# oKatanaaa/Cython3DModelRenderer

Measured on NVIDIA B200. Metric: T-Rex 1024^2 frames/s, higher is better.
Workload: dtype f32

## Files before the change

cython3dmodelrenderer_b200/csrc/crender_b200.cu:

```cuda

#include <cuda.h>
#include <cuda_runtime.h>

#include <climits>
#include <cmath>
#include <cstdarg>
#include <cstdint>
#include <cstdio>
#include <cstdlib>
#include <cstring>
#include <new>
#include <atomic>
#include <mutex>
#include <thread>
#include <vector>

#include "crender_b200.h"

namespace {

constexpr int TW = 32;
constexpr int TH = 32;
constexpr int NT = 256;
#ifndef CRB_RT
// ... 205 lines not shown
    c[2] = (X.w * b1 + C1.z * b2) + C2.y * b3;
    if (F.flags & CRB_GURO) {
        const float dot = (__fadd_rn(0.0f, n[0] * F.light[0]) + n[1] * F.light[1]) + n[2] * F.light[2];
        const float nrm = sqrtf((n[0] * n[0] + n[1] * n[1]) + n[2] * n[2]);
        float s = dot / (nrm + 1e-6f);
        if (s < 0.0f) s = 0.0f;
        if (s > 1.0f) s = 1.0f;
        c[0] *= s; c[1] *= s; c[2] *= s;
    }
    return true;
}

__device__ __forceinline__ float background_color(const Frame &)
{
    return 0.0f;
}

__device__ __forceinline__ unsigned char to_u8(float c)
{
    return (unsigned char)(c >= -2147483648.0f && c < 2147483648.0f ? (int)c : INT_MIN);
}

__device__ __forceinline__ unsigned char *u8_pixel(const Frame &F, int view, int yl, int x)
{
    const int fr = F.row1 - F.row0 - 1 - yl;
    if (F.u8xN) {
        const int d = fr / F.u8xRows;
        return F.u8x[d] + (((long long)view * F.u8xRows + (fr - d * F.u8xRows)) * F.W + x) * 3;
    }
    return F.color_u8 + ((long long)view * F.slabPixels + (long long)fr * F.W + x) * 3;
}


__device__ __forceinline__ void stage_floats(const float *__restrict__ g, long long first, long long count, float *s)
{
    const float *src = g + first;
    if (count == (long long)NT * 9 && (reinterpret_cast<uintptr_t>(src) & 15u) == 0) {
        const float4 *s4 = reinterpret_cast<const float4 *>(src);
        const unsigned t = threadIdx.x;
        const float4 a = __ldg(s4 + t), b = __ldg(s4 + t + NT);
        float4 c = make_float4(0.f, 0.f, 0.f, 0.f);
        if (t < NT * 9 / 4 - 2 * NT) c = __ldg(s4 + t + 2 * NT);
        reinterpret_cast<float4 *>(s)[t] = a;
        reinterpret_cast<float4 *>(s)[t + NT] = b;
        if (t < NT * 9 / 4 - 2 * NT) reinterpret_cast<float4 *>(s)[t + 2 * NT] = c;
    } else if ((reinterpret_cast<uintptr_t>(src) & 15u) == 0) {
        const long long n4 = count >> 2;
        const float4 *s4 = reinterpret_cast<const float4 *>(src);
        for (long long i = threadIdx.x; i < n4; i += NT) reinterpret_cast<float4 *>(s)[i] = __ldg(s4 + i);
        for (long long i = (n4 << 2) + threadIdx.x; i < count; i += NT) s[i] = __ldg(src + i);
    } else {
        for (long long i = threadIdx.x; i < count; i += NT) s[i] = __ldg(src + i);
    }
}

__device__ __forceinline__ void tile_span(const Frame &F, unsigned bx, unsigned by, int &tx0, int &tx1, int &ty0, int &ty1)
{
    const int xl = bx & 0xFFFF, xr = bx >> 16, yt = by & 0xFFFF, yb = by >> 16;
    tx0 = xl / TW;
    tx1 = (xr - 1) / TW;
    ty0 = (yt - F.row0) / TH;
    ty1 = (yb - 1 - F.row0) / TH;
}

constexpr int BC_STAGES = 4;
constexpr unsigned BC_BYTES = NT * 9 * 4;

__device__ __forceinline__ void mbar_init(unsigned long long *bar, unsigned count)
{
    asm volatile("mbarrier.init.shared::cta.b64 [%0], %1;" ::"r"((unsigned)__cvta_generic_to_shared(bar)), "r"(count) : "memory");
}
__device__ __forceinline__ void mbar_wait(unsigned long long *bar, unsigned phase)
{
    const unsigned a = (unsigned)__cvta_generic_to_shared(bar);
    asm volatile(
        "{\n"
        ".reg .pred p;\n"
        "WAIT_%=:\n"
        "mbarrier.try_wait.parity.shared::cta.b64 p, [%0], %1;\n"
        "@p bra DONE_%=;\n"
        "bra WAIT_%=;\n"
        "DONE_%=:\n"
        "}\n" ::"r"(a), "r"(phase) : "memory");
}
__device__ __forceinline__ void bulk_load(void *smem_dst, const void *gmem_src, unsigned bytes, unsigned long long *bar)
{
    const unsigned d = (unsigned)__cvta_generic_to_shared(smem_dst), m = (unsigned)__cvta_generic_to_shared(bar);
    asm volatile("mbarrier.arrive.expect_tx.shared::cta.b64 _, [%0], %1;" ::"r"(m), "r"(bytes) : "memory");
    asm volatile("cp.async.bulk.shared::cluster.global.mbarrier::complete_tx::bytes [%0], [%1], %2, [%3];" ::"r"(d), "l"(gmem_src),
                 "r"(bytes), "r"(m) : "memory");
}

__device__ __forceinline__ unsigned block_compact(const bool flag, unsigned *wsum, unsigned &total)
{
    const unsigned lane = threadIdx.x & 31u, wid = threadIdx.x >> 5;
    const unsigned b = __ballot_sync(0xFFFFFFFFu, flag);
    if (lane == 0) wsum[wid] = __popc(b);
    __syncthreads();
    unsigned base = 0, tot = 0;
#pragma unroll
    for (int w = 0; w < NT / 32; ++w) {
        const unsigned c = wsum[w];
        if (w < (int)wid) base += c;
        tot += c;
    }
    total = tot;
    __syncthreads();
    return base + __popc(b & ((1u << lane) - 1u));
}

__device__ __forceinline__ void setup_chunk(const Frame &F, const int view, const long long chunk, const long long chunksPerView,
                                            float *sv, float *sn, float *sc, float *sM, unsigned char *slist, unsigned *wsum,
                                            const bool staged)
{
    const long long first = chunk * NT;
    const long long cnt = min((long long)NT, F.T - first);
    const bool banded = F.row0 > 0 || F.row1 < F.H;
    unsigned short *alive = F.alive + (long long)view * chunksPerView + chunk;
    if (!staged) {
        stage_floats(F.v, first * 9, cnt * 9, sv);
        if (!banded) stage_floats(F.n, first * 9, cnt * 9, sn);
    }
    if (F.views && threadIdx.x < 16) sM[threadIdx.x] = F.views[view * 16 + threadIdx.x];
    __syncthreads();
    int me = threadIdx.x < cnt ? (int)threadIdx.x : -1;
    unsigned kept = 0;
    if (!banded) {
        bool keep = false;
        if (me >= 0) {
            const float *q = sn + me * 9;
            float z0 = q[2], z1 = q[5], z2 = q[8];
            if (F.views) {
                z0 = (sM[6] * q[0] + sM[7] * q[1]) + sM[8] * q[2];
                z1 = (sM[6] * q[3] + sM[7] * q[4]) + sM[8] * q[5];
                z2 = (sM[6] * q[6] + sM[7] * q[7]) + sM[8] * q[8];
            }
            keep = !(((z0 + z1) + z2) >= 0.0f);
        }
        const unsigned pos = block_compact(keep, wsum, kept);
        if (kept == 0) {
            if (threadIdx.x == 0) *alive = 0;
            return;
        }
        if (keep) slist[pos] = (unsigned char)me;
        __syncthreads();
        me = threadIdx.x < kept ? (int)slist[threadIdx.x] : -1;
    }
    const bool valid = me >= 0;
    const int mi = valid ? me : 0;
    const long long tri = first + mi;
    const long long ridx = (long long)view * F.T + tri;
    float x[3], y[3], z[3];
#pragma unroll
    for (int k = 0; k < 3; ++k) {
        if (!valid) { x[k] = y[k] = z[k] = 1.0f; continue; }
        x[k] = sv[mi * 9 + k * 3 + 0];
        y[k] = sv[mi * 9 + k * 3 + 1];
        z[k] = sv[mi * 9 + k * 3 + 2];
        if (F.views) view_point(sM, x[k], y[k], z[k]);
        project_vertex(F.proj, x[k], y[k], z[k]);
    }

    float fxl = (float)F.W, fxr = 0.0f, fyt = (float)F.H, fyb = 0.0f;
#pragma unroll
    for (int k = 0; k < 3; ++k) {
        if (x[k] < fxl) fxl = x[k];
        if (x[k] > fxr) fxr = x[k];
        if (y[k] < fyt) fyt = y[k];
        if (y[k] > fyb) fyb = y[k];
    }
    int xl = clipi(ceil_to_int_ref(fxl), 0, F.W), xr = clipi(ceil_to_int_ref(fxr), 0, F.W);
    int yt = clipi(ceil_to_int_ref(fyt), 0, F.H), yb = clipi(ceil_to_int_ref(fyb), 0, F.H);
    yt = max(yt, F.row0);
    yb = min(yb, F.row1);
    bool drawn = valid && (xl < xr) && (yt < yb);
    if (banded) {
        if (!__syncthreads_or(drawn ? 1 : 0)) {
            if (threadIdx.x == 0) *alive = 0;
            return;
        }
        if (!staged) {
            stage_floats(F.n, first * 9, cnt * 9, sn);
            __syncthreads();
        }
    }
    if (banded && valid) {
        const float *q = sn + mi * 9;
        float z0 = q[2], z1 = q[5], z2 = q[8];
        if (F.views) {
            z0 = (sM[6] * q[0] + sM[7] * q[1]) + sM[8] * q[2];
            z1 = (sM[6] * q[3] + sM[7] * q[4]) + sM[8] * q[5];
            z2 = (sM[6] * q[6] + sM[7] * q[7]) + sM[8] * q[8];
        }
        drawn = drawn && !(((z0 + z1) + z2) >= 0.0f);
    }
    const unsigned bx = drawn ? ((unsigned)xl | ((unsigned)xr << 16)) : 0u;
    const unsigned by = drawn ? ((unsigned)yt | ((unsigned)yb << 16)) : 0u;

    float l03 = 0.f, l13 = 0.f, l23 = 0.f;
    unsigned fl = 0;
    if (drawn) {
    l03 = (x[1] - x[2]) * (y[0] - y[2]) - (y[1] - y[2]) * (x[0] - x[2]);
    l13 = (x[2] - x[0]) * (y[1] - y[0]) - (y[2] - y[0]) * (x[1] - x[0]);
    l23 = (x[0] - x[1]) * (y[2] - y[1]) - (y[0] - y[1]) * (x[2] - x[1]);
    const float a03 = fabsf(l03), a13 = fabsf(l13), a23 = fabsf(l23);
    if (a03 >= L3_MIN && a03 <= L3_MAX) fl |= (FL_REJ << 0) | (l03 < 0.f ? (FL_NEG << 0) : 0u);
    if (a13 >= L3_MIN && a13 <= L3_MAX) fl |= (FL_REJ << 1) | (l13 < 0.f ? (FL_NEG << 1) : 0u);
    if (a23 >= L3_MIN && a23 <= L3_MAX) fl |= (FL_REJ << 2) | (l23 < 0.f ? (FL_NEG << 2) : 0u);
    float cmax = 0.0f;
#pragma unroll
    for (int k = 0; k < 3; ++k) cmax = fmaxf(cmax, fmaxf(fabsf(x[k]), fabsf(y[k])));
    const bool finite_xy = (x[0] - x[0] == 0.f) && (x[1] - x[1] == 0.f) && (x[2] - x[2] == 0.f) && (y[0] - y[0] == 0.f) &&
                           (y[1] - y[1] == 0.f) && (y[2] - y[2] == 0.f);
    if ((fl & (7u * FL_REJ)) == 7u * FL_REJ && finite_xy && cmax <= SPAN_COORD_MAX) fl |= FL_SPAN;
    if (fminf(fminf(a03, a13), a23) >= FDIV_LO && fmaxf(fmaxf(a03, a13), a23) <= FDIV_HI) fl |= FL_FDIV;
    }

    unsigned n_entries, dpos;
    bool entry;
    if (banded) {
        dpos = block_compact(drawn, wsum, n_entries);
        entry = drawn;
    } else {
        dpos = threadIdx.x; entry = valid;
        n_entries = __syncthreads_or(drawn ? 1 : 0) ? kept : 0u;
    }
    if (entry && n_entries) F.recE[(long long)view * F.T + first + dpos] = make_float4(__uint_as_float(bx), __uint_as_float(by), __uint_as_float((unsigned)mi), __uint_as_float(fl));
    if (threadIdx.x == 0) *alive = (unsigned short)n_entries;
    if (n_entries == 0) return;
    if (!staged) {
        stage_floats(F.c, first * 9, cnt * 9, sc);
        __syncthreads();
    }
    if (drawn) {
    float4 *R = F.shrec + ridx * SREC;
    const float *q = sc + mi * 9;
    R[S_A] = make_float4(x[0], y[0], x[1], y[1]);
    R[S_B] = make_float4(x[2], y[2], z[0], z[1]);
    R[S_C] = make_float4(z[2], l03, l13, l23);
    float nx[3], ny[3], nz[3];
#pragma unroll
    for (int k = 0; k < 3; ++k) {
        nx[k] = sn[mi * 9 + k * 3 + 0];
        ny[k] = sn[mi * 9 + k * 3 + 1];
        nz[k] = sn[mi * 9 + k * 3 + 2];
        if (F.views) view_normal(sM, nx[k], ny[k], nz[k]);
    }
    R[S_N0] = make_float4(nx[0], ny[0], nz[0], nx[1]);
    R[S_N1] = make_float4(ny[1], nz[1], nx[2], ny[2]);
    R[S_X] = make_float4(nz[2], q[0], q[1], q[2]);
    R[S_C1] = make_float4(q[3], q[4], q[5], q[6]);
    R[S_C2] = make_float4(q[7], q[8], __uint_as_float(fl), 0.0f);
    }
    if (F.flags & CRB_PATH_ATOMIC) return;

    int tx0 = 0, tx1 = -1, ty0 = 0, ty1 = -1;
    if (drawn) tile_span(F, bx, by, tx0, tx1, ty0, ty1);
    unsigned *cnt_view = F.count + (long long)view * F.nTiles;
    const int nt = drawn ? (tx1 - tx0 + 1) * (ty1 - ty0 + 1) : 0;
    if (nt <= WIDE_TILES)
        for (int ty = ty0; ty <= ty1; ++ty)
            for (int tx = tx0; tx <= tx1; ++tx) atomicAdd(cnt_view + ty * F.tilesX + tx, 1u);
    for (unsigned wide = __ballot_sync(0xFFFFFFFFu, nt > WIDE_TILES); wide; wide &= wide - 1u) {
        const int src = __ffs(wide) - 1;
        const int sx0 = __shfl_sync(0xFFFFFFFFu, tx0, src), sx1 = __shfl_sync(0xFFFFFFFFu, tx1, src);
        const int sy0 = __shfl_sync(0xFFFFFFFFu, ty0, src), n = __shfl_sync(0xFFFFFFFFu, nt, src);
        const int wx = sx1 - sx0 + 1;
        for (int i = (int)(threadIdx.x & 31u); i < n; i += 32) atomicAdd(cnt_view + (sy0 + i / wx) * F.tilesX + sx0 + i % wx, 1u);
    }
}

#ifndef CRB_SETUP_MIN_CTAS
#define CRB_SETUP_MIN_CTAS 3
#endif
constexpr int SETUP_STAGES = 2;
constexpr size_t SETUP_STAGE_FLOATS = 3 * (size_t)NT * 9;
constexpr size_t SETUP_DYN_SMEM = SETUP_STAGES * SETUP_STAGE_FLOATS * sizeof(float);
__global__ void __launch_bounds__(NT, CRB_SETUP_MIN_CTAS) k_setup(const Frame F)
{
    extern __shared__ __align__(128) float stg[];
    __shared__ __align__(8) unsigned long long bar[SETUP_STAGES];
    __shared__ float sM[16];
    __shared__ unsigned char slist[NT];
    __shared__ unsigned wsum[NT / 32];
    if (blockIdx.x == 0 && threadIdx.x == 0) {
        F.total[0] = 0ull; F.total[2] = 0ull; F.total[3] = 0ull; F.total[4] = 0ull; F.total[5] = 0ull;
    }
    const long long chunksPerView = (F.T + NT - 1) / NT;
    const long long nItems = F.chunks ? (long long)F.chunks[0] : chunksPerView * F.nViews;
    const bool banded = F.row0 > 0 || F.row1 < F.H;
    const bool bulk_ok = !((reinterpret_cast<uintptr_t>(F.v) | reinterpret_cast<uintptr_t>(F.n) | reinterpret_cast<uintptr_t>(F.c)) & 15u) &&
                         (!banded || F.chunks);
    auto item = [&](long long w, int &view) -> long long {
        if (F.chunks) { view = 0; return (long long)F.chunks[1 + w]; }
        view = (int)(w / chunksPerView);
        return w % chunksPerView;
    };
    auto issue = [&](long long w, int s) {
        int view;
        const long long chunk = item(w, view);
        if (!bulk_ok || (chunk + 1) * NT > F.T) return;
        float *d = stg + (size_t)s * SETUP_STAGE_FLOATS;
        bulk_load(d, F.v + chunk * NT * 9, BC_BYTES, &bar[s]);
        bulk_load(d + NT * 9, F.n + chunk * NT * 9, BC_BYTES, &bar[s]);
        bulk_load(d + 2 * NT * 9, F.c + chunk * NT * 9, BC_BYTES, &bar[s]);
    };
    if (threadIdx.x == 0) {
        for (int s = 0; s < SETUP_STAGES; ++s) mbar_init(&bar[s], 3u);
        asm volatile("fence.mbarrier_init.release.cluster;" ::: "memory");
        for (int s = 0; s < SETUP_STAGES; ++s)
            if ((long long)blockIdx.x + (long long)s * gridDim.x < nItems) issue((long long)blockIdx.x + (long long)s * gridDim.x, s);
    }
    __syncthreads();
    unsigned uses = 0;
    int i = 0;
    for (long long w = blockIdx.x; w < nItems; w += gridDim.x, ++i) {
        const int s = i % SETUP_STAGES;
        int view;
        const long long chunk = item(w, view);
        const bool staged = bulk_ok && (chunk + 1) * NT <= F.T;
        if (staged) {
            mbar_wait(&bar[s], (uses >> s) & 1u);
            uses ^= 1u << s;
        }
        float *d = stg + (size_t)s * SETUP_STAGE_FLOATS;
        setup_chunk(F, view, chunk, chunksPerView, d, d + NT * 9, d + 2 * NT * 9, sM, slist, wsum, staged);
        __syncthreads();
        const long long w2 = w + (long long)SETUP_STAGES * gridDim.x;
        if (threadIdx.x == 0 && w2 < nItems) issue(w2, s);
    }
}

__global__ void __launch_bounds__(NT) k_band_chunks(const Frame F)
{
    __shared__ __align__(128) float sv[BC_STAGES][NT * 9];
    __shared__ __align__(8) unsigned long long bar[BC_STAGES];
    const long long nFull = F.T / NT;
    if (blockIdx.x == 0 && threadIdx.x == 0 && nFull * NT < F.T) F.chunks[1 + atomicAdd(F.chunks, 1u)] = (unsigned)nFull;
    const long long nMine = nFull > blockIdx.x ? (nFull - blockIdx.x + gridDim.x - 1) / gridDim.x : 0;
    if (threadIdx.x == 0) {
        for (int s = 0; s < BC_STAGES; ++s) mbar_init(&bar[s], 1u);
        asm volatile("fence.mbarrier_init.release.cluster;" ::: "memory");
        for (int j = 0; j < BC_STAGES && j < nMine; ++j)
            bulk_load(sv[j], F.v + (blockIdx.x + (long long)j * gridDim.x) * (NT * 9), BC_BYTES, &bar[j]);
    }
    __syncthreads();
    for (long long j = 0; j < nMine; ++j) {
        const int s = (int)(j % BC_STAGES);
        mbar_wait(&bar[s], (unsigned)((j / BC_STAGES) & 1));
        float ylo = 3.0e38f, yhi = -3.0e38f;
        bool odd = false;
#pragma unroll
        for (int k = 0; k < 3; ++k) {
            const float vx = sv[s][threadIdx.x * 9 + k * 3 + 0];
            const float vy = sv[s][threadIdx.x * 9 + k * 3 + 1];
            const float vz = sv[s][threadIdx.x * 9 + k * 3 + 2];
            const float X = ((vx * F.proj.p[0] + vy * F.proj.p[4]) + vz * F.proj.p[8]) + F.proj.p[12];
            const float Y = ((X * F.proj.p[1] + vy * F.proj.p[5]) + vz * F.proj.p[9]) + F.proj.p[13];
            float r;
            asm("rcp.approx.ftz.f32 %0, %1;" : "=f"(r) : "f"(vz));
            const float ysc = (Y * r + 1.0f) * F.proj.ys;
            if (!(fabsf(ysc) < 1.0e9f)) odd = true;
// ... 52 lines not shown
    unsigned nheavyTiles;
    const unsigned htile = block_exclusive_scan(heavy ? 1u : 0u, warp_sums, nheavyTiles);
    __shared__ unsigned heavy_base;
    if (threadIdx.x == 0) {
        const unsigned valid = (unsigned)min((long long)NT, nAll - (long long)blockIdx.x * NT);
        block_base = tot ? atomicAdd(F.total, (unsigned long long)tot) : 0ull;
        busy_base = (unsigned)atomicAdd(F.total + 2, (unsigned long long)(nbusy - nheavyTiles));
        heavy_base = (unsigned)atomicAdd(F.total + 4, (unsigned long long)nheavy);
        empty_base = (unsigned)atomicAdd(F.total + 3, (unsigned long long)(valid - nbusy));
    }
    __syncthreads();
    if (i < nAll) {
        const unsigned long long o = block_base + excl;
        const unsigned o32 = (unsigned)(o > 0xFFFFFFFFull ? 0xFFFFFFFFull : o);
        F.offset[i] = o32;
        F.cursor[i] = 0u;
        F.count[i] = 0u;
        const unsigned vw = (unsigned)(i / F.nTiles), tl = (unsigned)(i % F.nTiles);
        const unsigned packed = (vw << 22) | ((tl / (unsigned)F.tilesX) << 11) | (tl % (unsigned)F.tilesX);
        constexpr unsigned FULL = (unsigned)TH << 8;
        if (cut)
            for (unsigned b = 0; b < (unsigned)SPLIT_BANDS; ++b)
                F.busyH[heavy_base + hrank + b] = make_uint4(packed, c, o32, (b * (TH / SPLIT_BANDS)) | (((b + 1) * (TH / SPLIT_BANDS)) << 8));
        else if (heavy) F.busyH[heavy_base + hrank] = make_uint4(packed, c, o32, FULL);
        else if (c) F.busy[busy_base + (brank - htile)] = make_uint4(packed, c, o32, FULL);
        else F.empty[empty_base + (threadIdx.x - brank)] = packed;
    }
}

constexpr int FT = 64;
__device__ __forceinline__ void fill_chunk(const Frame &F, const int view, const long long chunk, const long long chunksPerView, const bool skip,
                                           const unsigned tix )
{
    const long long slot = chunk * NT + tix;
    const float4 E = slot < F.T ? F.recE[(long long)view * F.T + slot] : make_float4(0.f, 0.f, 0.f, 0.f);
    const unsigned nd = F.alive[(long long)view * chunksPerView + chunk];
    if (skip || (tix & ~31u) >= nd) return;
    const unsigned bx = tix < nd ? __float_as_uint(E.x) : 0u, by = tix < nd ? __float_as_uint(E.y) : 0u;
    const bool drawn = (bx >> 16) != 0;
    const long long tri = chunk * NT + (drawn ? (long long)(__float_as_uint(E.z) & 255u) : 0ll);
    const long long ridx = (long long)view * F.T + tri;
    float4 a = make_float4(0.f, 0.f, 0.f, 0.f), b = a, s2 = a, s3 = a;
    int tx0 = 0, tx1 = -1, ty0 = 0, ty1 = -1;
    if (drawn) {
        const float4 *R = F.shrec + ridx * SREC;
        const float4 c = R[S_C];
        a = R[S_A]; b = R[S_B];
        const unsigned fl = __float_as_uint(E.w);
        s2 = make_float4(c.x, (fl & (FL_NEG << 0)) ? -c.y : c.y, (fl & (FL_NEG << 1)) ? -c.z : c.z, (fl & (FL_NEG << 2)) ? -c.w : c.w);
        s3 = make_float4(__uint_as_float(bx), __uint_as_float(by), __uint_as_float((unsigned)tri), __uint_as_float(fl));
        tile_span(F, bx, by, tx0, tx1, ty0, ty1);
    }
    const long long vb = (long long)view * F.nTiles;
    const int nt = drawn ? (tx1 - tx0 + 1) * (ty1 - ty0 + 1) : 0;
    {
        const unsigned lane = tix & 31u;
        const int small = nt <= WIDE_TILES ? nt : 0;
        const int turns = __reduce_max_sync(0xFFFFFFFFu, small);
        int cx = tx0, cy = ty0;
        for (int k = 0; k < turns; ++k) {
            const bool act = k < small;
            const long long t = vb + cy * F.tilesX + cx;
            const unsigned tag = act ? (unsigned)t : 0xFFFFFFE0u + lane;
            const unsigned grp = __match_any_sync(0xFFFFFFFFu, tag);
            const int leader = __ffs(grp) - 1;
            unsigned base = 0;
            if (act && (int)lane == leader) base = F.offset[t] + atomicAdd(F.cursor + t, (unsigned)__popc(grp));
            base = __shfl_sync(0xFFFFFFFFu, base, leader);
            if (act) {
                float4 *o = F.ls + (size_t)(base + __popc(grp & ((1u << lane) - 1u))) * 4;
                o[0] = a; o[1] = b; o[2] = s2; o[3] = s3;
                if (++cx > tx1) { cx = tx0; ++cy; }
            }
        }
    }
    unsigned widem = __ballot_sync(0xFFFFFFFFu, nt > WIDE_TILES);
    if (F.wideCap && widem) {
        const unsigned lane = tix & 31u;
        unsigned long long first = 0ull;
        if ((int)lane == __ffs(widem) - 1) first = atomicAdd(F.total + 5, (unsigned long long)__popc(widem));
        first = __shfl_sync(0xFFFFFFFFu, first, __ffs(widem) - 1);
        const unsigned long long at = first + __popc(widem & ((1u << lane) - 1u));
        const bool listed = nt > WIDE_TILES && at < (unsigned long long)F.wideCap;
        if (listed) F.wide[at] = make_uint4((unsigned)view, (unsigned)tri, bx, by);
        widem = __ballot_sync(0xFFFFFFFFu, nt > WIDE_TILES && !listed);
    }
    for (unsigned wide = widem; wide; wide &= wide - 1u) {
        const int src = __ffs(wide) - 1;
        auto bc = [src](float4 v) {
            return make_float4(__shfl_sync(0xFFFFFFFFu, v.x, src), __shfl_sync(0xFFFFFFFFu, v.y, src), __shfl_sync(0xFFFFFFFFu, v.z, src),
                               __shfl_sync(0xFFFFFFFFu, v.w, src));
        };
        const float4 wa = bc(a), wb = bc(b), w2 = bc(s2), w3 = bc(s3);
        const int sx0 = __shfl_sync(0xFFFFFFFFu, tx0, src), sx1 = __shfl_sync(0xFFFFFFFFu, tx1, src);
        const int sy0 = __shfl_sync(0xFFFFFFFFu, ty0, src), n = __shfl_sync(0xFFFFFFFFu, nt, src);
        const int wx = sx1 - sx0 + 1;
        for (int i = (int)(tix & 31u); i < n; i += 32) {
            const long long t = vb + (sy0 + i / wx) * F.tilesX + sx0 + i % wx;
            const unsigned at = F.offset[t] + atomicAdd(F.cursor + t, 1u);
            float4 *o = F.ls + (size_t)at * 4;
            o[0] = wa; o[1] = wb; o[2] = w2; o[3] = w3;
        }
    }
}

#ifndef CRB_FILL_MIN_CTAS
#define CRB_FILL_MIN_CTAS 16
#endif
__global__ void __launch_bounds__(FT, CRB_FILL_MIN_CTAS) k_fill(const Frame F)
{
    const long long chunksPerView = (F.T + NT - 1) / NT;
    const unsigned tix = (blockIdx.x & (NT / FT - 1)) * FT + threadIdx.x;
    if (!F.chunks) {
        fill_chunk(F, blockIdx.y, blockIdx.x / (NT / FT), chunksPerView, *F.total > (unsigned long long)F.pairCap, tix);
        return;
    }
    if (*F.total > (unsigned long long)F.pairCap) return;
    const unsigned n = F.chunks[0];
    for (unsigned i = blockIdx.x / (NT / FT); i < n; i += gridDim.x / (NT / FT)) fill_chunk(F, 0, F.chunks[1 + i], chunksPerView, false, tix);
}

constexpr int FWT = 256;
__global__ void __launch_bounds__(FWT) k_fill_wide(const Frame F)
{
    if (*F.total > (unsigned long long)F.pairCap) return;
    const unsigned long long listed = F.total[5];
    const unsigned n = (unsigned)(listed < (unsigned long long)F.wideCap ? listed : (unsigned long long)F.wideCap);
    for (unsigned e = blockIdx.x; e < n; e += gridDim.x) {
        const uint4 w = F.wide[e];
        const long long ridx = (long long)w.x * F.T + w.y;
        const float4 *R = F.shrec + ridx * SREC;
        const float4 a = R[S_A], b = R[S_B], c = R[S_C];
        const unsigned fl = __float_as_uint(R[S_C2].z);
        const float4 s2 = make_float4(c.x, (fl & (FL_NEG << 0)) ? -c.y : c.y, (fl & (FL_NEG << 1)) ? -c.z : c.z, (fl & (FL_NEG << 2)) ? -c.w : c.w);
        const float4 s3 = make_float4(__uint_as_float(w.z), __uint_as_float(w.w), __uint_as_float(w.y), __uint_as_float(fl));
        int tx0, tx1, ty0, ty1;
        tile_span(F, w.z, w.w, tx0, tx1, ty0, ty1);
        const int wx = tx1 - tx0 + 1, nt = wx * (ty1 - ty0 + 1);
        const long long vb = (long long)w.x * F.nTiles;
        for (int i0 = (int)threadIdx.x; i0 < nt; i0 += 4 * FWT) {
// ... 561 lines not shown

#ifdef CRB_LARGE_OUT_STAGE
constexpr bool LARGE_OUT_STAGE = true;
#else
constexpr bool LARGE_OUT_STAGE = false;
#endif
typedef RasterShape<CRB_RT, CRB_CH, CRB_FQ, CRB_CLEAR_ROWS, CRB_RASTER_MIN_CTAS, LARGE_OUT_STAGE> RasterLarge;
#ifndef CRB_SMALL_RT
#define CRB_SMALL_RT 128
#endif
#ifndef CRB_SMALL_CH
#define CRB_SMALL_CH 24
#endif
#ifndef CRB_SMALL_FQ
#define CRB_SMALL_FQ 256
#endif
#ifndef CRB_SMALL_CLEAR_ROWS
#define CRB_SMALL_CLEAR_ROWS 8
#endif
#ifndef CRB_SMALL_MIN_CTAS
#define CRB_SMALL_MIN_CTAS 12
#endif
typedef RasterShape<CRB_SMALL_RT, CRB_SMALL_CH, CRB_SMALL_FQ, CRB_SMALL_CLEAR_ROWS, CRB_SMALL_MIN_CTAS, false> RasterSmall;
typedef RasterShape<256, 128, 256, 16, 6, false> RasterWide;
#ifndef CRB_SHAPE_LARGE_FROM
#define CRB_SHAPE_LARGE_FROM 64
#endif

__global__ void __launch_bounds__(NT) k_raster_atomic(const Frame F, unsigned long long *keybuf)
{
    const long long slot = ((long long)blockIdx.x * NT + threadIdx.x) >> 5;
    const int lane = threadIdx.x & 31;
    if (slot >= F.T || (unsigned)(slot % NT) >= F.alive[slot / NT]) return;
    const float4 r2 = F.recE[slot];
    const unsigned bx = __float_as_uint(r2.x), by = __float_as_uint(r2.y);
    if ((bx >> 16) == 0) return;
    const long long tri = slot / NT * NT + (__float_as_uint(r2.z) & 255u);
    const Tri9 t = load_tri9(F, tri);
    const int xl = bx & 0xFFFF, xr = bx >> 16, yt = by & 0xFFFF, yb = by >> 16;
    const int bw = xr - xl;
    const long long area = (long long)bw * (yb - yt);
    for (long long i = lane; i < area; i += 32) {
        const int x = xl + (int)(i % bw), y = yt + (int)(i / bw);
        float b1, b2, b3;
        barycentric(t, (float)x, (float)y, b1, b2, b3);
        if (b1 < 0.0f || b2 < 0.0f || b3 < 0.0f) continue;
        const float z = (t.z0 * b1 + t.z1 * b2) + t.z2 * b3;
        if (z != z) continue;
        atomicMin(keybuf + (long long)(y - F.row0) * F.W + x, pack_key(z, (unsigned)tri));
    }
}

__global__ void __launch_bounds__(NT) k_shade_atomic(const Frame F, unsigned long long *keybuf)
{
    const long long pix = (long long)blockIdx.x * NT + threadIdx.x;
    if (pix >= F.slabPixels) return;
    const unsigned long long key = keybuf[pix];
    const bool clear = (F.flags & CRB_CLEAR_FIRST) != 0;
    float z = Z_INIT, c[3] = {0.f, 0.f, 0.f}, nn[3] = {0.f, 0.f, 0.f};
    bool write = clear;
    if (key != KEY_EMPTY) {
        keybuf[pix] = KEY_EMPTY;
        const unsigned tri = ~(unsigned)(key & 0xFFFFFFFFull);
        const int y = F.row0 + (int)(pix / F.W), x = (int)(pix % F.W);
        float fz, fc[3], fn[3];
        if (shade_fragment(F, F.shrec + (size_t)tri * SREC, (float)x, (float)y, fz, fc, fn)) {
            const float zold = clear ? Z_INIT : F.z[pix];
            if (!(fz > zold)) {
                z = fz; c[0] = fc[0]; c[1] = fc[1]; c[2] = fc[2]; nn[0] = fn[0]; nn[1] = fn[1]; nn[2] = fn[2];
                write = true;
// ... 249 lines not shown
    unsigned long long *hstats;
    unsigned long long *hstats_dev;
    bool prof_on;
    int prof_n;
    cudaEvent_t *prof_ev;
    int wide_kernel;
    unsigned char *u8x[CRB_MAX_EXCHANGE];
    int u8x_n, u8x_rows;
};

namespace {

struct WsLayout {
    size_t shrec, recE, alive, chunks, count, offset, cursor, busy, busyH, empty, ls, wide, total, set_bytes, sv, sc, sn, bytes;
};

long long default_pair_cap(const crb_filler *f, long long T, int views)
{
    const long long tiles = (long long)((f->w + TW - 1) / TW) * ((f->row1 - f->row0 + TH - 1) / TH);
    long long cap = 4 * T * views + tiles * views + 65536;
    return cap;
}

long long wide_capacity(long long T, int views) { return (T > 0 ? T : 1) * views / 8 + 1024; }

WsLayout ws_layout(const crb_filler *f, long long T, int views, long long pairCap)
{
    WsLayout L;
    const long long tiles = (long long)((f->w + TW - 1) / TW) * ((f->row1 - f->row0 + TH - 1) / TH);
    size_t o = 0;
    auto take = [&](size_t bytes) { size_t at = o; o = align_up(o + bytes, 256); return at; };
    const size_t recs = (size_t)(T > 0 ? T : 1) * views;
    L.shrec = take(recs * SREC * sizeof(float4));
    L.recE = take(recs * sizeof(float4));
    L.alive = take((size_t)((T > 0 ? T : 1) + NT - 1) / NT * views * sizeof(unsigned short));
    L.chunks = take(4 * ((size_t)((T > 0 ? T : 1) + NT - 1) / NT + 2));
    L.count = take((size_t)tiles * views * 4);
    L.offset = take((size_t)tiles * views * 4);
    L.cursor = take((size_t)tiles * views * 4);
    L.busy = take((size_t)tiles * views * 16);
    L.busyH = take((size_t)tiles * views * 16 * SPLIT_BANDS);
    L.empty = take((size_t)tiles * views * 4);
    L.ls = take((size_t)pairCap * 64);
    L.wide = take((size_t)wide_capacity(T, views) * 16);
    L.total = take(64);
    L.set_bytes = o;
    o = 2 * L.set_bytes;
    L.sv = take((size_t)(T > 0 ? T : 1) * 36);
    L.sc = take((size_t)(T > 0 ? T : 1) * 36);
    L.sn = take((size_t)(T > 0 ? T : 1) * 36);
    L.bytes = o;
    return L;
}

int check_filler(const crb_filler *f)
{
    if (!f) return fail(CRB_ERR_INVALID, "filler is NULL");
    return CRB_OK;
}

int check_triangles(const crb_filler *f, int64_t T, const float *v, const float *c, const float *n)
{
    if (T < 0) return fail(CRB_ERR_INVALID, "T < 0");
    if (T > 0 && (!v || !c || !n)) return fail(CRB_ERR_INVALID, "NULL triangle array");
    if (!f->ws) return fail(CRB_ERR_STATE, "workspace not bound");
    if (T > f->maxT) return fail(CRB_ERR_STATE, "T=%lld exceeds the workspace's max_triangles=%lld", (long long)T, f->maxT);
    if (T > 0xFFFFFFF0ll) return fail(CRB_ERR_INVALID, "T exceeds 32-bit triangle indices");
// ... 103 lines not shown
    return CRB_OK;
}

#ifndef CRB_PREPASS_EIGHTHS
#define CRB_PREPASS_EIGHTHS 5
#endif
int run_prep(crb_filler *f, Frame &F, cudaStream_t st, int slot = 0)
{
    int rc;
    bool wide_kernel = false;
    if (f->hstats && f->wide_kernel) {
        const unsigned long long hs = *reinterpret_cast<volatile unsigned long long *>(f->hstats + HSTAT_WORDS * (slot & 7));
        const unsigned long long hw = *reinterpret_cast<volatile unsigned long long *>(f->hstats + HSTAT_WORDS * (slot & 7) + 1) >> 32;
        wide_kernel = hs == 0ull || hw >= 24ull * (unsigned long long)F.nViews;
    }
    F.wideCap = wide_kernel && !(F.flags & CRB_PATH_ATOMIC) ? (unsigned)(f->wideCap > 0xFFFFFFF0ll ? 0xFFFFFFF0ll : f->wideCap) : 0u;
    unsigned gT = (unsigned)((F.T + NT - 1) / NT);
    const bool banded = F.row0 > 0 || F.row1 < F.H;
    F.chunks = nullptr;
    if (banded && f->band_prepass && 8ll * (F.row1 - F.row0) <= (long long)CRB_PREPASS_EIGHTHS * F.H && F.nViews == 1 && !F.views && F.T >= 8 * NT && !(F.flags & CRB_PATH_ATOMIC) &&
        !(reinterpret_cast<uintptr_t>(F.v) & 15u)) {
        const size_t so = (size_t)(reinterpret_cast<const char *>(F.alive) - reinterpret_cast<const char *>(f->alive));
        F.chunks = reinterpret_cast<unsigned *>(reinterpret_cast<char *>(f->chunks) + so);
        CU(cudaMemsetAsync(F.chunks, 0, 4, st));
        constexpr int bcPerSm = 4;
        const unsigned gP = (unsigned)min((long long)gT, (long long)f->sm_count * bcPerSm);
        k_band_chunks<<<gP, NT, 0, st>>>(F);
        if ((rc = launch_check(f, "k_band_chunks"))) return rc;
        gT = (unsigned)min((long long)gT, (long long)f->sm_count * 6);
    }
    if (F.T > 0) {
        if ((rc = setup_smem_attr(f->device))) return rc;
        const long long items = F.chunks ? (long long)gT : (long long)gT * F.nViews;
        k_setup<<<(unsigned)min(items, (long long)f->sm_count * CRB_SETUP_MIN_CTAS), NT, SETUP_DYN_SMEM, st>>>(F);
        if ((rc = launch_check(f, "k_setup"))) return rc;
    } else {
        CU(cudaMemsetAsync(F.total, 0, 8, st));
        CU(cudaMemsetAsync(F.total + 2, 0, 24, st));
    }
    F.splitHeavy = (F.nViews == 1 && f->split_heavy && F.nTiles <= 4 * f->sm_count * 6) ? 1u : 0u;
    const long long nAllTiles = (long long)F.nViews * F.nTiles;
    k_alloc<<<(unsigned)((nAllTiles + NT - 1) / NT), NT, 0, st>>>(F);
    if ((rc = launch_check(f, "k_alloc"))) return rc;
    if (F.T > 0) {
        k_fill<<<dim3(gT * (NT / FT), F.nViews), FT, 0, st>>>(F);
        if ((rc = launch_check(f, "k_fill"))) return rc;
        if (F.wideCap) {
            k_fill_wide<<<(unsigned)f->sm_count * 6, FWT, 0, st>>>(F);
            if ((rc = launch_check(f, "k_fill_wide"))) return rc;
        }
    }
    return CRB_OK;
}

int run_raster(crb_filler *f, Frame &F, cudaStream_t st, int slot)
{
    int rc;
    slot &= 7;
    if (F.hstats) F.hstats += HSTAT_WORDS * slot;
    const long long nAllTiles = (long long)F.nViews * F.nTiles;
    const bool prof = f->prof_on && f->prof_n < PROF_MAX;
    int shape = f->raster_shape;
    if (shape == 0) {
        const long long wave = (long long)f->sm_count * RasterWide::MIN_CTAS;
        double busy = (double)nAllTiles, per_tile = (double)F.T * 2.0 / (double)F.nTiles;
        if (f->hstats) {
            const unsigned long long hs = *reinterpret_cast<volatile unsigned long long *>(f->hstats + HSTAT_WORDS * slot);
// ... 39 lines not shown
    if (prof) CU(cudaEventRecord(f->prof_ev[2 * f->prof_n], st));
    if (shape == 2) k_raster<RasterSmall><<<(unsigned)gR, RasterSmall::RT, 0, st>>>(F, M);
    else if (shape == 3) k_raster<RasterWide><<<(unsigned)gR, RasterWide::RT, 0, st>>>(F, M);
    else k_raster<RasterLarge><<<(unsigned)gR, RasterLarge::RT, 0, st>>>(F, M);
    if ((rc = launch_check(f, "k_raster"))) return rc;
    if (prof) {
        CU(cudaEventRecord(f->prof_ev[2 * f->prof_n + 1], st));
        f->prof_n++;
    }
    return CRB_OK;
}

int run_tiled(crb_filler *f, Frame &F, cudaStream_t st, int slot = 0)
{
    int rc = run_prep(f, F, st, slot);
    return rc ? rc : run_raster(f, F, st, slot);
}

int run_atomic(crb_filler *f, Frame &F, cudaStream_t st)
{
    int rc;
    if (F.nViews != 1 || F.views) return fail(CRB_ERR_INVALID, "CRB_PATH_ATOMIC supports single-view renders only");
    if (!F.z || !F.color || !F.normals) return fail(CRB_ERR_STATE, "CRB_PATH_ATOMIC needs all three buffers");
    if (f->keybuf_pixels < F.slabPixels) {
        if (f->keybuf) cudaFree(f->keybuf);
        f->keybuf = nullptr;
        CU(cudaMalloc(&f->keybuf, (size_t)F.slabPixels * 8));
        f->keybuf_pixels = F.slabPixels;
        k_fill_u64<<<1184, NT, 0, st>>>(f->keybuf, F.slabPixels, KEY_EMPTY);
        if ((rc = launch_check(f, "k_fill_u64"))) return rc;
    }
    if (F.T > 0) {
        if ((rc = setup_smem_attr(f->device))) return rc;
        k_setup<<<(unsigned)min((F.T + NT - 1) / NT, (long long)f->sm_count * CRB_SETUP_MIN_CTAS), NT, SETUP_DYN_SMEM, st>>>(F);
        if ((rc = launch_check(f, "k_setup"))) return rc;
        k_raster_atomic<<<(unsigned)((F.T * 32 + NT - 1) / NT), NT, 0, st>>>(F, f->keybuf);
        if ((rc = launch_check(f, "k_raster_atomic"))) return rc;
    }
    k_shade_atomic<<<(unsigned)((F.slabPixels + NT - 1) / NT), NT, 0, st>>>(F, f->keybuf);
    return launch_check(f, "k_shade_atomic");
}

int join_pending(crb_filler *f, cudaStream_t st)
{
    if (f->pending_join) {
        CU(cudaStreamWaitEvent(st, f->ev_raster[f->pending_join - 1], 0));
        f->pending_join = 0;
    }
    return CRB_OK;
}

int bind_ws_pointers(crb_filler *f, void *ws, size_t bytes, long long T, int views, long long pairCap, cudaStream_t st)
{
    if (views < 1) views = 1;
    if (views > 1024) return fail(CRB_ERR_INVALID, "max_views > 1024 (views per launch; crb_render_views chunks longer batches itself)");
    if (T < 0) return fail(CRB_ERR_INVALID, "max_triangles < 0");
    if (pairCap <= 0) pairCap = default_pair_cap(f, T, views);
    if (pairCap > 0xFFFFFFF0ll) return fail(CRB_ERR_INVALID, "pair capacity exceeds 32-bit list offsets");
    const WsLayout L = ws_layout(f, T, views, pairCap);
    if (!ws || bytes < L.bytes) return fail(CRB_ERR_INVALID, "workspace too small: %zu < %zu", bytes, L.bytes);
    if (reinterpret_cast<uintptr_t>(ws) & 255u) return fail(CRB_ERR_INVALID, "workspace must be 256-byte aligned");
    char *b = (char *)ws;
    f->ws = ws; f->ws_bytes = bytes;
    f->maxT = T; f->maxViews = views; f->pairCap = pairCap;
    f->shrec = (float4 *)(b + L.shrec); f->recE = (float4 *)(b + L.recE);
    f->alive = (unsigned short *)(b + L.alive);
    f->chunks = (unsigned *)(b + L.chunks);
// ... 906 lines not shown
```

Baseline: 129,300.

## Restructure setup kernel into warp-independent culling with compact fat fill records

The setup kernel moves to 128-thread blocks in which each warp culls and sets up 64 triangles on its own. Block-wide compaction and __syncthreads are replaced by warp ballots plus a shared atomic counter, and the last warp to finish refills the stage. Color is no longer bulk-staged and is read directly from global memory. Setup now writes a 4-float4 compacted record holding geometry and the global triangle index, so the fill and atomic kernels read it directly instead of gathering from shrec. This removes block barriers and gather indirection, at the cost of a 4x larger recE buffer, more global writes, and reordered entry slots (the atomic order is nondeterministic).

```diff
diff --git a/cython3dmodelrenderer_b200/csrc/crender_b200.cu b/cython3dmodelrenderer_b200/csrc/crender_b200.cu
--- a/cython3dmodelrenderer_b200/csrc/crender_b200.cu
+++ b/cython3dmodelrenderer_b200/csrc/crender_b200.cu
@@ -261,28 +261,6 @@
 }
 
 
-__device__ __forceinline__ void stage_floats(const float *__restrict__ g, long long first, long long count, float *s)
-{
-    const float *src = g + first;
-    if (count == (long long)NT * 9 && (reinterpret_cast<uintptr_t>(src) & 15u) == 0) {
-        const float4 *s4 = reinterpret_cast<const float4 *>(src);
-        const unsigned t = threadIdx.x;
-        const float4 a = __ldg(s4 + t), b = __ldg(s4 + t + NT);
-        float4 c = make_float4(0.f, 0.f, 0.f, 0.f);
-        if (t < NT * 9 / 4 - 2 * NT) c = __ldg(s4 + t + 2 * NT);
-        reinterpret_cast<float4 *>(s)[t] = a;
-        reinterpret_cast<float4 *>(s)[t + NT] = b;
-        if (t < NT * 9 / 4 - 2 * NT) reinterpret_cast<float4 *>(s)[t + 2 * NT] = c;
-    } else if ((reinterpret_cast<uintptr_t>(src) & 15u) == 0) {
-        const long long n4 = count >> 2;
-        const float4 *s4 = reinterpret_cast<const float4 *>(src);
-        for (long long i = threadIdx.x; i < n4; i += NT) reinterpret_cast<float4 *>(s)[i] = __ldg(s4 + i);
-        for (long long i = (n4 << 2) + threadIdx.x; i < count; i += NT) s[i] = __ldg(src + i);
-    } else {
-        for (long long i = threadIdx.x; i < count; i += NT) s[i] = __ldg(src + i);
-    }
-}
-
 __device__ __forceinline__ void tile_span(const Frame &F, unsigned bx, unsigned by, int &tx0, int &tx1, int &ty0, int &ty1)
 {
     const int xl = bx & 0xFFFF, xr = bx >> 16, yt = by & 0xFFFF, yb = by >> 16;
@@ -312,69 +290,30 @@
         "DONE_%=:\n"
         "}\n" ::"r"(a), "r"(phase) : "memory");
 }
-__device__ __forceinline__ void bulk_load(void *smem_dst, const void *gmem_src, unsigned bytes, unsigned long long *bar)
+__device__ __forceinline__ void mbar_arrive(unsigned long long *bar)
+{
+    asm volatile("mbarrier.arrive.shared::cta.b64 _, [%0];" ::"r"((unsigned)__cvta_generic_to_shared(bar)) : "memory");
+}
+__device__ __forceinline__ void mbar_arrive_expect_tx(unsigned long long *bar, unsigned bytes)
+{
+    asm volatile("mbarrier.arrive.expect_tx.shared::cta.b64 _, [%0], %1;" ::"r"((unsigned)__cvta_generic_to_shared(bar)), "r"(bytes) : "memory");
+}
+__device__ __forceinline__ void bulk_copy(void *smem_dst, const void *gmem_src, unsigned bytes, unsigned long long *bar)
 {
     const unsigned d = (unsigned)__cvta_generic_to_shared(smem_dst), m = (unsigned)__cvta_generic_to_shared(bar);
-    asm volatile("mbarrier.arrive.expect_tx.shared::cta.b64 _, [%0], %1;" ::"r"(m), "r"(bytes) : "memory");
     asm volatile("cp.async.bulk.shared::cluster.global.mbarrier::complete_tx::bytes [%0], [%1], %2, [%3];" ::"r"(d), "l"(gmem_src),
                  "r"(bytes), "r"(m) : "memory");
 }
-
-__device__ __forceinline__ unsigned block_compact(const bool flag, unsigned *wsum, unsigned &total)
-{
-    const unsigned lane = threadIdx.x & 31u, wid = threadIdx.x >> 5;
-    const unsigned b = __ballot_sync(0xFFFFFFFFu, flag);
-    if (lane == 0) wsum[wid] = __popc(b);
-    __syncthreads();
-    unsigned base = 0, tot = 0;
-#pragma unroll
-    for (int w = 0; w < NT / 32; ++w) {
-        const unsigned c = wsum[w];
-        if (w < (int)wid) base += c;
-        tot += c;
-    }
-    total = tot;
-    __syncthreads();
-    return base + __popc(b & ((1u << lane) - 1u));
-}
-
-__device__ __forceinline__ void setup_chunk(const Frame &F, const int view, const long long chunk, const long long chunksPerView,
-                                            float *sv, float *sn, float *sc, float *sM, unsigned char *slist, unsigned *wsum,
-                                            const bool staged)
-{
-    const long long first = chunk * NT;
-    const long long cnt = min((long long)NT, F.T - first);
-    const bool banded = F.row0 > 0 || F.row1 < F.H;
-    unsigned short *alive = F.alive + (long long)view * chunksPerView + chunk;
-    if (!staged) {
-        stage_floats(F.v, first * 9, cnt * 9, sv);
-        if (!banded) stage_floats(F.n, first * 9, cnt * 9, sn);
-    }
-    if (F.views && threadIdx.x < 16) sM[threadIdx.x] = F.views[view * 16 + threadIdx.x];
-    __syncthreads();
-    int me = threadIdx.x < cnt ? (int)threadIdx.x : -1;
-    unsigned kept = 0;
-    if (!banded) {
-        bool keep = false;
-        if (me >= 0) {
-            const float *q = sn + me * 9;
-            float z0 = q[2], z1 = q[5], z2 = q[8];
-            if (F.views) {
-                z0 = (sM[6] * q[0] + sM[7] * q[1]) + sM[8] * q[2];
-                z1 = (sM[6] * q[3] + sM[7] * q[4]) + sM[8] * q[5];
-                z2 = (sM[6] * q[6] + sM[7] * q[7]) + sM[8] * q[8];
-            }
-            keep = !(((z0 + z1) + z2) >= 0.0f);
-        }
-        const unsigned pos = block_compact(keep, wsum, kept);
-        if (kept == 0) {
-            if (threadIdx.x == 0) *alive = 0;
-            return;
-        }
-        if (keep) slist[pos] = (unsigned char)me;
-        __syncthreads();
-        me = threadIdx.x < kept ? (int)slist[threadIdx.x] : -1;
-    }
+__device__ __forceinline__ void bulk_load(void *smem_dst, const void *gmem_src, unsigned bytes, unsigned long long *bar)
+{
+    mbar_arrive_expect_tx(bar, bytes);
+    bulk_copy(smem_dst, gmem_src, bytes, bar);
+}
+
+__device__ __forceinline__ void setup_tri(const Frame &F, const int view, const long long first, const int me, const bool banded,
+                                          const float *sv, const float *sn, const float *sM, unsigned *ecount)
+{
+    const unsigned lane = threadIdx.x & 31u;
     const bool valid = me >= 0;
     const int mi = valid ? me : 0;
     const long long tri = first + mi;
@@ -403,17 +342,7 @@
     yt = max(yt, F.row0);
     yb = min(yb, F.row1);
     bool drawn = valid && (xl < xr) && (yt < yb);
-    if (banded) {
-        if (!__syncthreads_or(drawn ? 1 : 0)) {
-            if (threadIdx.x == 0) *alive = 0;
-            return;
-        }
-        if (!staged) {
-            stage_floats(F.n, first * 9, cnt * 9, sn);
-            __syncthreads();
-        }
-    }
-    if (banded && valid) {
+    if (banded && drawn) {
         const float *q = sn + mi * 9;
         float z0 = q[2], z1 = q[5], z2 = q[8];
         if (F.views) {
@@ -421,8 +350,10 @@
             z1 = (sM[6] * q[3] + sM[7] * q[4]) + sM[8] * q[5];
             z2 = (sM[6] * q[6] + sM[7] * q[7]) + sM[8] * q[8];
         }
-        drawn = drawn && !(((z0 + z1) + z2) >= 0.0f);
-    }
+        drawn = !(((z0 + z1) + z2) >= 0.0f);
+    }
+    const unsigned dm = __ballot_sync(0xFFFFFFFFu, drawn);
+    if (dm == 0u) return;
     const unsigned bx = drawn ? ((unsigned)xl | ((unsigned)xr << 16)) : 0u;
     const unsigned by = drawn ? ((unsigned)yt | ((unsigned)yb << 16)) : 0u;
 
@@ -445,25 +376,16 @@
     if (fminf(fminf(a03, a13), a23) >= FDIV_LO && fmaxf(fmaxf(a03, a13), a23) <= FDIV_HI) fl |= FL_FDIV;
     }
 
-    unsigned n_entries, dpos;
-    bool entry;
-    if (banded) {
-        dpos = block_compact(drawn, wsum, n_entries);
-        entry = drawn;
-    } else {
-        dpos = threadIdx.x; entry = valid;
-        n_entries = __syncthreads_or(drawn ? 1 : 0) ? kept : 0u;
-    }
-    if (entry && n_entries) F.recE[(long long)view * F.T + first + dpos] = make_float4(__uint_as_float(bx), __uint_as_float(by), __uint_as_float((unsigned)mi), __uint_as_float(fl));
-    if (threadIdx.x == 0) *alive = (unsigned short)n_entries;
-    if (n_entries == 0) return;
-    if (!staged) {
-        stage_floats(F.c, first * 9, cnt * 9, sc);
-        __syncthreads();
-    }
+    unsigned base = 0;
+    if (lane == 0) base = atomicAdd(ecount, (unsigned)__popc(dm));
+    base = __shfl_sync(0xFFFFFFFFu, base, 0);
     if (drawn) {
+    float4 *E = F.recE + ((long long)view * F.T + first + base + __popc(dm & ((1u << lane) - 1u))) * 4;
+    E[0] = make_float4(x[0], y[0], x[1], y[1]);
+    E[1] = make_float4(x[2], y[2], z[0], z[1]);
+    E[2] = make_float4(z[2], (fl & (FL_NEG << 0)) ? -l03 : l03, (fl & (FL_NEG << 1)) ? -l13 : l13, (fl & (FL_NEG << 2)) ? -l23 : l23);
+    E[3] = make_float4(__uint_as_float(bx), __uint_as_float(by), __uint_as_float((unsigned)tri), __uint_as_float(fl));
     float4 *R = F.shrec + ridx * SREC;
-    const float *q = sc + mi * 9;
     R[S_A] = make_float4(x[0], y[0], x[1], y[1]);
     R[S_B] = make_float4(x[2], y[2], z[0], z[1]);
     R[S_C] = make_float4(z[2], l03, l13, l23);
@@ -475,11 +397,12 @@
         nz[k] = sn[mi * 9 + k * 3 + 2];
         if (F.views) view_normal(sM, nx[k], ny[k], nz[k]);
     }
+    const float *q = F.c + tri * 9;
     R[S_N0] = make_float4(nx[0], ny[0], nz[0], nx[1]);
     R[S_N1] = make_float4(ny[1], nz[1], nx[2], ny[2]);
-    R[S_X] = make_float4(nz[2], q[0], q[1], q[2]);
-    R[S_C1] = make_float4(q[3], q[4], q[5], q[6]);
-    R[S_C2] = make_float4(q[7], q[8], __uint_as_float(fl), 0.0f);
+    R[S_X] = make_float4(nz[2], __ldg(q + 0), __ldg(q + 1), __ldg(q + 2));
+    R[S_C1] = make_float4(__ldg(q + 3), __ldg(q + 4), __ldg(q + 5), __ldg(q + 6));
+    R[S_C2] = make_float4(__ldg(q + 7), __ldg(q + 8), __uint_as_float(fl), 0.0f);
     }
     if (F.flags & CRB_PATH_ATOMIC) return;
 
@@ -495,68 +418,131 @@
         const int sx0 = __shfl_sync(0xFFFFFFFFu, tx0, src), sx1 = __shfl_sync(0xFFFFFFFFu, tx1, src);
         const int sy0 = __shfl_sync(0xFFFFFFFFu, ty0, src), n = __shfl_sync(0xFFFFFFFFu, nt, src);
         const int wx = sx1 - sx0 + 1;
-        for (int i = (int)(threadIdx.x & 31u); i < n; i += 32) atomicAdd(cnt_view + (sy0 + i / wx) * F.tilesX + sx0 + i % wx, 1u);
+        for (int i = (int)lane; i < n; i += 32) atomicAdd(cnt_view + (sy0 + i / wx) * F.tilesX + sx0 + i % wx, 1u);
+    }
+}
+
+constexpr int ST = 128;
+constexpr int SETUP_WARPS = ST / 32;
+constexpr int SETUP_TPW = NT / SETUP_WARPS;
+static_assert(SETUP_TPW == 64, "setup_chunk culls two triangles per lane");
+
+__device__ __forceinline__ void setup_chunk(const Frame &F, const int view, const long long first, const int cnt, const float *sv,
+                                            const float *sn, const float *sM, unsigned char *sl, unsigned *ecount)
+{
+    const unsigned lane = threadIdx.x & 31u;
+    const int wbase = (int)(threadIdx.x >> 5) * SETUP_TPW;
+    const bool banded = F.row0 > 0 || F.row1 < F.H;
+    int k;
+    if (banded) {
+        k = clipi(cnt - wbase, 0, SETUP_TPW);
+    } else {
+        bool keep[2];
+#pragma unroll
+        for (int h = 0; h < 2; ++h) {
+            const int me = wbase + h * 32 + (int)lane;
+            keep[h] = false;
+            if (me < cnt) {
+                const float *q = sn + me * 9;
+                float z0 = q[2], z1 = q[5], z2 = q[8];
+                if (F.views) {
+                    z0 = (sM[6] * q[0] + sM[7] * q[1]) + sM[8] * q[2];
+                    z1 = (sM[6] * q[3] + sM[7] * q[4]) + sM[8] * q[5];
+                    z2 = (sM[6] * q[6] + sM[7] * q[7]) + sM[8] * q[8];
+                }
+                keep[h] = !(((z0 + z1) + z2) >= 0.0f);
+            }
+        }
+        const unsigned m0 = __ballot_sync(0xFFFFFFFFu, keep[0]), m1 = __ballot_sync(0xFFFFFFFFu, keep[1]);
+        const unsigned lt = (1u << lane) - 1u;
+        if (keep[0]) sl[__popc(m0 & lt)] = (unsigned char)(wbase + lane);
+        if (keep[1]) sl[__popc(m0) + __popc(m1 & lt)] = (unsigned char)(wbase + 32 + lane);
+        __syncwarp();
+        k = __popc(m0) + __popc(m1);
+    }
+    for (int p = 0; p < k; p += 32) {
+        const int j = p + (int)lane;
+        const int me = j < k ? (banded ? wbase + j : (int)sl[j]) : -1;
+        setup_tri(F, view, first, me, banded, sv, sn, sM, ecount);
     }
 }
 
 #ifndef CRB_SETUP_MIN_CTAS
-#define CRB_SETUP_MIN_CTAS 3
+#define CRB_SETUP_MIN_CTAS 6
 #endif
 constexpr int SETUP_STAGES = 2;
-constexpr size_t SETUP_STAGE_FLOATS = 3 * (size_t)NT * 9;
+constexpr size_t SETUP_STAGE_FLOATS = 2 * (size_t)NT * 9;
 constexpr size_t SETUP_DYN_SMEM = SETUP_STAGES * SETUP_STAGE_FLOATS * sizeof(float);
-__global__ void __launch_bounds__(NT, CRB_SETUP_MIN_CTAS) k_setup(const Frame F)
+__global__ void __launch_bounds__(ST, CRB_SETUP_MIN_CTAS) k_setup(const Frame F)
 {
     extern __shared__ __align__(128) float stg[];
-    __shared__ __align__(8) unsigned long long bar[SETUP_STAGES];
-    __shared__ float sM[16];
-    __shared__ unsigned char slist[NT];
-    __shared__ unsigned wsum[NT / 32];
+    __shared__ __align__(8) unsigned long long full[SETUP_STAGES];
+    __shared__ unsigned ecount[SETUP_STAGES], done[SETUP_STAGES];
+    __shared__ float sM[SETUP_WARPS][16];
+    __shared__ unsigned char sl[SETUP_WARPS][SETUP_TPW];
     if (blockIdx.x == 0 && threadIdx.x == 0) {
         F.total[0] = 0ull; F.total[2] = 0ull; F.total[3] = 0ull; F.total[4] = 0ull; F.total[5] = 0ull;
     }
     const long long chunksPerView = (F.T + NT - 1) / NT;
     const long long nItems = F.chunks ? (long long)F.chunks[0] : chunksPerView * F.nViews;
     const bool banded = F.row0 > 0 || F.row1 < F.H;
-    const bool bulk_ok = !((reinterpret_cast<uintptr_t>(F.v) | reinterpret_cast<uintptr_t>(F.n) | reinterpret_cast<uintptr_t>(F.c)) & 15u) &&
-                         (!banded || F.chunks);
+    const bool bulk_ok = !((reinterpret_cast<uintptr_t>(F.v) | reinterpret_cast<uintptr_t>(F.n)) & 15u) && (!banded || F.chunks);
     auto item = [&](long long w, int &view) -> long long {
         if (F.chunks) { view = 0; return (long long)F.chunks[1 + w]; }
         view = (int)(w / chunksPerView);
         return w % chunksPerView;
     };
-    auto issue = [&](long long w, int s) {
+    auto staged = [&](long long chunk) { return bulk_ok && (chunk + 1) * NT <= F.T; };
+    auto refill = [&](long long w, int s) {
         int view;
         const long long chunk = item(w, view);
-        if (!bulk_ok || (chunk + 1) * NT > F.T) return;
+        if (!staged(chunk)) { mbar_arrive(&full[s]); return; }
         float *d = stg + (size_t)s * SETUP_STAGE_FLOATS;
-        bulk_load(d, F.v + chunk * NT * 9, BC_BYTES, &bar[s]);
-        bulk_load(d + NT * 9, F.n + chunk * NT * 9, BC_BYTES, &bar[s]);
-        bulk_load(d + 2 * NT * 9, F.c + chunk * NT * 9, BC_BYTES, &bar[s]);
+        mbar_arrive_expect_tx(&full[s], 2 * BC_BYTES);
+        bulk_copy(d, F.v + chunk * NT * 9, BC_BYTES, &full[s]);
+        bulk_copy(d + NT * 9, F.n + chunk * NT * 9, BC_BYTES, &full[s]);
     };
     if (threadIdx.x == 0) {
-        for (int s = 0; s < SETUP_STAGES; ++s) mbar_init(&bar[s], 3u);
+        for (int s = 0; s < SETUP_STAGES; ++s) {
+            mbar_init(&full[s], 1u);
+            ecount[s] = 0u;
+            done[s] = 0u;
+        }
         asm volatile("fence.mbarrier_init.release.cluster;" ::: "memory");
         for (int s = 0; s < SETUP_STAGES; ++s)
-            if ((long long)blockIdx.x + (long long)s * gridDim.x < nItems) issue((long long)blockIdx.x + (long long)s * gridDim.x, s);
+            if ((long long)blockIdx.x + (long long)s * gridDim.x < nItems) refill((long long)blockIdx.x + (long long)s * gridDim.x, s);
     }
     __syncthreads();
+    const unsigned lane = threadIdx.x & 31u, wid = threadIdx.x >> 5;
     unsigned uses = 0;
     int i = 0;
     for (long long w = blockIdx.x; w < nItems; w += gridDim.x, ++i) {
         const int s = i % SETUP_STAGES;
         int view;
         const long long chunk = item(w, view);
-        const bool staged = bulk_ok && (chunk + 1) * NT <= F.T;
-        if (staged) {
-            mbar_wait(&bar[s], (uses >> s) & 1u);
-            uses ^= 1u << s;
-        }
-        float *d = stg + (size_t)s * SETUP_STAGE_FLOATS;
-        setup_chunk(F, view, chunk, chunksPerView, d, d + NT * 9, d + 2 * NT * 9, sM, slist, wsum, staged);
-        __syncthreads();
-        const long long w2 = w + (long long)SETUP_STAGES * gridDim.x;
-        if (threadIdx.x == 0 && w2 < nItems) issue(w2, s);
+        mbar_wait(&full[s], (uses >> s) & 1u);
+        uses ^= 1u << s;
+        if (F.views && lane < 16) sM[wid][lane] = F.views[view * 16 + lane];
+        __syncwarp();
+        const long long first = chunk * NT;
+        const int cnt = (int)min((long long)NT, F.T - first);
+        if (staged(chunk)) {
+            const float *d = stg + (size_t)s * SETUP_STAGE_FLOATS;
+            setup_chunk(F, view, first, cnt, d, d + NT * 9, sM[wid], sl[wid], &ecount[s]);
+        } else {
+            setup_chunk(F, view, first, cnt, F.v + first * 9, F.n + first * 9, sM[wid], sl[wid], &ecount[s]);
+        }
+        __syncwarp();
+        if (lane == 0) {
+            __threadfence_block();
+            if (atomicAdd(&done[s], 1u) == SETUP_WARPS - 1) {
+                __threadfence_block();
+                F.alive[(long long)view * chunksPerView + chunk] = (unsigned short)atomicExch(&ecount[s], 0u);
+                done[s] = 0u;
+                const long long w2 = w + (long long)SETUP_STAGES * gridDim.x;
+                if (w2 < nItems) refill(w2, s);
+            }
+        }
     }
 }
 
@@ -675,24 +661,15 @@
 __device__ __forceinline__ void fill_chunk(const Frame &F, const int view, const long long chunk, const long long chunksPerView, const bool skip,
                                            const unsigned tix )
 {
-    const long long slot = chunk * NT + tix;
-    const float4 E = slot < F.T ? F.recE[(long long)view * F.T + slot] : make_float4(0.f, 0.f, 0.f, 0.f);
     const unsigned nd = F.alive[(long long)view * chunksPerView + chunk];
     if (skip || (tix & ~31u) >= nd) return;
-    const unsigned bx = tix < nd ? __float_as_uint(E.x) : 0u, by = tix < nd ? __float_as_uint(E.y) : 0u;
-    const bool drawn = (bx >> 16) != 0;
-    const long long tri = chunk * NT + (drawn ? (long long)(__float_as_uint(E.z) & 255u) : 0ll);
-    const long long ridx = (long long)view * F.T + tri;
+    const bool drawn = tix < nd;
     float4 a = make_float4(0.f, 0.f, 0.f, 0.f), b = a, s2 = a, s3 = a;
     int tx0 = 0, tx1 = -1, ty0 = 0, ty1 = -1;
     if (drawn) {
-        const float4 *R = F.shrec + ridx * SREC;
-        const float4 c = R[S_C];
-        a = R[S_A]; b = R[S_B];
-        const unsigned fl = __float_as_uint(E.w);
-        s2 = make_float4(c.x, (fl & (FL_NEG << 0)) ? -c.y : c.y, (fl & (FL_NEG << 1)) ? -c.z : c.z, (fl & (FL_NEG << 2)) ? -c.w : c.w);
-        s3 = make_float4(__uint_as_float(bx), __uint_as_float(by), __uint_as_float((unsigned)tri), __uint_as_float(fl));
-        tile_span(F, bx, by, tx0, tx1, ty0, ty1);
+        const float4 *E = F.recE + ((long long)view * F.T + chunk * NT + tix) * 4;
+        a = E[0]; b = E[1]; s2 = E[2]; s3 = E[3];
+        tile_span(F, __float_as_uint(s3.x), __float_as_uint(s3.y), tx0, tx1, ty0, ty1);
     }
     const long long vb = (long long)view * F.nTiles;
     const int nt = drawn ? (tx1 - tx0 + 1) * (ty1 - ty0 + 1) : 0;
@@ -725,16 +702,13 @@
         first = __shfl_sync(0xFFFFFFFFu, first, __ffs(widem) - 1);
         const unsigned long long at = first + __popc(widem & ((1u << lane) - 1u));
         const bool listed = nt > WIDE_TILES && at < (unsigned long long)F.wideCap;
-        if (listed) F.wide[at] = make_uint4((unsigned)view, (unsigned)tri, bx, by);
+        if (listed) F.wide[at] = make_uint4((unsigned)view, __float_as_uint(s3.z), __float_as_uint(s3.x), __float_as_uint(s3.y));
         widem = __ballot_sync(0xFFFFFFFFu, nt > WIDE_TILES && !listed);
     }
     for (unsigned wide = widem; wide; wide &= wide - 1u) {
         const int src = __ffs(wide) - 1;
-        auto bc = [src](float4 v) {
-            return make_float4(__shfl_sync(0xFFFFFFFFu, v.x, src), __shfl_sync(0xFFFFFFFFu, v.y, src), __shfl_sync(0xFFFFFFFFu, v.z, src),
-                               __shfl_sync(0xFFFFFFFFu, v.w, src));
-        };
-        const float4 wa = bc(a), wb = bc(b), w2 = bc(s2), w3 = bc(s3);
+        const float4 *W = F.recE + ((long long)view * F.T + chunk * NT + (tix & ~31u) + src) * 4;
+        const float4 wa = W[0], wb = W[1], w2 = W[2], w3 = W[3];
         const int sx0 = __shfl_sync(0xFFFFFFFFu, tx0, src), sx1 = __shfl_sync(0xFFFFFFFFu, tx1, src);
         const int sy0 = __shfl_sync(0xFFFFFFFFu, ty0, src), n = __shfl_sync(0xFFFFFFFFu, nt, src);
         const int wx = sx1 - sx0 + 1;
@@ -748,7 +722,7 @@
 }
 
 #ifndef CRB_FILL_MIN_CTAS
-#define CRB_FILL_MIN_CTAS 16
+#define CRB_FILL_MIN_CTAS 20
 #endif
 __global__ void __launch_bounds__(FT, CRB_FILL_MIN_CTAS) k_fill(const Frame F)
 {
@@ -1376,10 +1350,9 @@
     const long long slot = ((long long)blockIdx.x * NT + threadIdx.x) >> 5;
     const int lane = threadIdx.x & 31;
     if (slot >= F.T || (unsigned)(slot % NT) >= F.alive[slot / NT]) return;
-    const float4 r2 = F.recE[slot];
+    const float4 r2 = F.recE[slot * 4 + 3];
     const unsigned bx = __float_as_uint(r2.x), by = __float_as_uint(r2.y);
-    if ((bx >> 16) == 0) return;
-    const long long tri = slot / NT * NT + (__float_as_uint(r2.z) & 255u);
+    const long long tri = __float_as_uint(r2.z);
     const Tri9 t = load_tri9(F, tri);
     const int xl = bx & 0xFFFF, xr = bx >> 16, yt = by & 0xFFFF, yb = by >> 16;
     const int bw = xr - xl;
@@ -1695,7 +1668,7 @@
     auto take = [&](size_t bytes) { size_t at = o; o = align_up(o + bytes, 256); return at; };
     const size_t recs = (size_t)(T > 0 ? T : 1) * views;
     L.shrec = take(recs * SREC * sizeof(float4));
-    L.recE = take(recs * sizeof(float4));
+    L.recE = take(recs * 4 * sizeof(float4));
     L.alive = take((size_t)((T > 0 ? T : 1) + NT - 1) / NT * views * sizeof(unsigned short));
     L.chunks = take(4 * ((size_t)((T > 0 ? T : 1) + NT - 1) / NT + 2));
     L.count = take((size_t)tiles * views * 4);
@@ -1865,7 +1838,7 @@
     if (F.T > 0) {
         if ((rc = setup_smem_attr(f->device))) return rc;
         const long long items = F.chunks ? (long long)gT : (long long)gT * F.nViews;
-        k_setup<<<(unsigned)min(items, (long long)f->sm_count * CRB_SETUP_MIN_CTAS), NT, SETUP_DYN_SMEM, st>>>(F);
+        k_setup<<<(unsigned)min(items, (long long)f->sm_count * CRB_SETUP_MIN_CTAS), ST, SETUP_DYN_SMEM, st>>>(F);
         if ((rc = launch_check(f, "k_setup"))) return rc;
     } else {
         CU(cudaMemsetAsync(F.total, 0, 8, st));
@@ -1971,7 +1944,7 @@
     }
     if (F.T > 0) {
         if ((rc = setup_smem_attr(f->device))) return rc;
-        k_setup<<<(unsigned)min((F.T + NT - 1) / NT, (long long)f->sm_count * CRB_SETUP_MIN_CTAS), NT, SETUP_DYN_SMEM, st>>>(F);
+        k_setup<<<(unsigned)min((F.T + NT - 1) / NT, (long long)f->sm_count * CRB_SETUP_MIN_CTAS), ST, SETUP_DYN_SMEM, st>>>(F);
         if ((rc = launch_check(f, "k_setup"))) return rc;
         k_raster_atomic<<<(unsigned)((F.T * 32 + NT - 1) / NT), NT, 0, st>>>(F, f->keybuf);
         if ((rc = launch_check(f, "k_raster_atomic"))) return rc;
```

Result: no change. 129,200 (median of 6 runs) (-0.1%).
